# ChanghyeonKim93/nonlinear_optimizer_for_slam

Measured on AMD Instinct MI355X. Metric: ndt6_gauss_newton_residual_blocks_per_sec, higher is better.
Workload: dtype f64

## Files before the change

### nonlinear_optimizer_for_slam_amd/csrc/assemble_indexed.hpp

```cpp
#pragma once

#include "assemble_one_launch.hpp"

namespace nos {

struct IndexedLayout {
  const void* points;
  const int32_t* index;
  const void* table;
  uint64_t n_padded;
};

template <typename T>
__device__ __forceinline__ void load_voxel_record(const T* table, int32_t v, T (&rec)[12]) {
  const T* p = table + size_t(16) * size_t(v);
  if constexpr (sizeof(T) == 8) {
    using V2 = double __attribute__((ext_vector_type(2)));
    const V2* q = reinterpret_cast<const V2*>(p);
#pragma unroll
    for (int k = 0; k < 4; ++k) {
      const V2 t = q[k];
      rec[2 * k] = t[0];
      rec[2 * k + 1] = t[1];
    }
// ... 44 lines not shown
  T pt[kPointRing][3];
  int32_t id[kPointRing][K];
  T rc[kRecordRing][K][12];
  auto evaluate = [&](bool live, const T (&p)[3], const int32_t (&vid)[K], const T (&rec)[K][12]) {
#pragma unroll
    for (int k = 0; k < K; ++k) {
      if (live && vid[k] >= 0) {
        const T mu[3] = {rec[k][0], rec[k][1], rec[k][2]};
        const T U[6] = {rec[k][3], rec[k][4], rec[k][5], rec[k][6], rec[k][7], rec[k][8]};
        Problem::item_U(p, mu, U, P, acc);
      }
    }
  };
  uint32_t c = blockIdx.x;
  const uint32_t g = gridDim.x;
#pragma unroll
  for (int s = 0; s < kPointAhead; ++s) load_point(c + uint32_t(s) * g, pt[s], id[s]);
  load_records(id[0], rc[0]);
  for (; c < n_chunks; c += uint32_t(kUnroll) * g) {
#pragma unroll
    for (int u = 0; u < kUnroll; ++u) {
      load_point(c + uint32_t(u + kPointAhead) * g, pt[(u + kPointAhead) % kPointRing], id[(u + kPointAhead) % kPointRing]);
      load_records(id[(u + 1) % kPointRing], rc[(u + 1) % kRecordRing]);
      __builtin_amdgcn_sched_barrier(0);
      evaluate(c + uint32_t(u) * g < n_chunks, pt[u % kPointRing], id[u % kPointRing], rc[u % kRecordRing]);
      __builtin_amdgcn_sched_barrier(0);
    }
  }
  double dacc[kOut];
#pragma unroll
  for (int k = 0; k < kOut; ++k) dacc[k] = double(acc[k]);
  block_reduce_store<kOut, BLOCK>(dacc, partials + size_t(blockIdx.x) * kOut, fin.write_through != 0);
  if (fin.counter != nullptr) finish_in_last_block<kOut, BLOCK>(partials, fin);
}

template <typename SRC, typename DST>
__global__ __launch_bounds__(256) void gather_plane_kernel(const SRC* __restrict__ src, const uint32_t* __restrict__ perm,
                                                           uint64_t n, uint64_t n_padded, DST pad_value,
                                                           DST* __restrict__ dst) {
  const uint64_t j = uint64_t(blockIdx.x) * 256 + threadIdx.x;
  if (j >= n_padded) return;
  dst[j] = j < n ? DST(src[perm ? perm[j] : j]) : pad_value;
}

template <typename T>
__global__ __launch_bounds__(256) void build_voxel_table_kernel(const double* __restrict__ means,
                                                                const double* __restrict__ sqrt_infos,
                                                                const uint32_t* __restrict__ rows, uint64_t n_voxels,
                                                                T* __restrict__ table) {
  const uint64_t t = uint64_t(blockIdx.x) * 256 + threadIdx.x;
  const uint64_t r = t >> 4;
  const int k = int(t & 15);
  if (r >= n_voxels) return;
  const uint64_t v = rows ? rows[r] : r;
  T val = T(0);
  if (k < 3) {
    val = T(means[3 * v + k]);
  } else if (k < 9) {
    double S[9], U[6];
#pragma unroll
    for (int q = 0; q < 9; ++q) S[q] = sqrt_infos[9 * v + q];
    sqrt_info_to_U<double>(S, U);
    const int q = k - 3;
    val = T(q == 0 ? U[0] : q == 1 ? U[1] : q == 2 ? U[2] : q == 3 ? U[3] : q == 4 ? U[4] : U[5]);
  }
  table[t] = val;
// ... 19 lines not shown
```

### nonlinear_optimizer_for_slam_amd/csrc/nos_core.hip

```cpp
#include "nos_internal.hpp"

namespace nosd {


thread_local const void* t_last_kernel = nullptr;

template <typename Problem, typename T, int ITEMS, int BLOCK, int MINW, int PREFETCH = 0>
int launch_variant(const nos::TiledLayout& L, const typename Problem::Params& P, int grid_cap, int num_cus_hint,
                   bool nt, double* partials, const nos::FusedFinal& fin_in, hipStream_t stream, int* rows_out) {
  constexpr uint32_t kChunk = BLOCK * ITEMS;
  if (L.n_padded % kChunk != 0) return fail(NOS_ERR_INVALID_ARGUMENT, "n_padded %% chunk != 0");
  if (L.tile_stride != 0 && ((size_t(L.tile_mask) + 1) % kChunk) != 0)
    return fail(NOS_ERR_INVALID_ARGUMENT, "tile not a multiple of the kernel chunk");
  const uint64_t n_chunks64 = L.n_padded / kChunk;
  if (n_chunks64 > 0xFFFFFFFFull) return fail(NOS_ERR_UNSUPPORTED, "dataset too large for one shard");
  const uint32_t n_chunks = uint32_t(n_chunks64);
  int grid = int(std::min<uint64_t>(n_chunks, uint64_t(grid_cap)));
  if (grid < 1) grid = 1;
  if (grid > kMaxPartialRows) grid = kMaxPartialRows;
  nos::FusedFinal fin = fin_in;
  fin.write_through = (fin.counter != nullptr && grid <= num_cus_hint && fin_in.write_through != 0) ? 1 : 0;
  const auto kernel = nt ? nos::assemble_kernel<Problem, T, ITEMS, BLOCK, MINW, true, PREFETCH>
                         : nos::assemble_kernel<Problem, T, ITEMS, BLOCK, MINW, false, PREFETCH>;
  t_last_kernel = reinterpret_cast<const void*>(kernel);
// ... 38 lines not shown
  } else {
    if (variant == 0) variant = kReproj ? 11 : 1;
    switch (variant) {
      NOS_CASE(1, 2, 512, 2, 1)
      NOS_CASE_PP(11, 2, 512, 2, 1)
#ifdef NOS_ALL_VARIANTS
      NOS_CASE(2, 1, 256, 4, 2)
      NOS_CASE(3, 2, 256, 5, 2)
      NOS_CASE(4, 2, 256, 4, 2)
      NOS_CASE(5, 1, 1024, 4, 1)
      NOS_CASE(6, 2, 1024, 4, 1)
      NOS_CASE(9, 2, 256, 3, 3)
      NOS_CASE_PP(12, 4, 512, 2, 1)
      NOS_CASE(13, 4, 256, 2, 1)
#endif
    }
  }
#undef NOS_CASE
#undef NOS_CASE_PP
  return fail(NOS_ERR_UNSUPPORTED, "launch geometry %d is not compiled into this build for this element type "
              "(default build: fp64 0, 1, 3, 7; fp32 1, 11; `make ALL_VARIANTS=1` builds the rest)", variant);
}

size_t resident_items_per_lane(int n_fields, int dtype) {
  if (n_fields == 15)
    return dtype == NOS_F64 ? size_t(nos::ResidentShape<15, 8>::RI + nos::ResidentShape<15, 8>::LI)
                            : size_t(nos::ResidentShape<15, 4>::RI + nos::ResidentShape<15, 4>::LI);
  if (n_fields == 5)
    return dtype == NOS_F64 ? size_t(nos::ResidentShape<5, 8>::RI + nos::ResidentShape<5, 8>::LI)
                            : size_t(nos::ResidentShape<5, 4>::RI + nos::ResidentShape<5, 4>::LI);
  return 1;
}

struct SingleBlockArgs {
  int cluster_blocks = 0;
  int items_per_lane = 1;
  int stream_chunks = 0;
  bool nt = false;
  int stream_lds_chunks = 0;
  int stream_reg_rounds = 0;
  bool stage1_sc1 = false;
  const nos::Mailbox* mail = nullptr;
  double* partials = nullptr;
  nos::ClusterCtl* ctl = nullptr;
  nos::LmDevice* lm;
  double* history;
  int history_capacity;
  double* entry;
  unsigned long long* seq_host;
  unsigned long long seq;
};

template <typename Problem, typename T>
int launch_single(const nos::TiledLayout& L, const typename Problem::Params& P, const SingleBlockArgs& a, hipStream_t stream) {
  constexpr int kBlock = 512;
  if (L.n_padded % kBlock != 0) return fail(NOS_ERR_INVALID_ARGUMENT, "n_padded %% 512 != 0");
  if (a.cluster_blocks > 0 && a.stream_chunks > 0) {
    constexpr int kSI = sizeof(T) == 8 ? 1 : 2;
    constexpr bool kSPF = false;
    constexpr size_t kChunk = size_t(kBlock) * kSI;
    if (L.n_padded % kChunk != 0 || (L.tile_stride != 0 && ((size_t(L.tile_mask) + 1) % kChunk) != 0))
      return fail(NOS_ERR_INVALID_ARGUMENT, "streaming solve: layout not a multiple of the %zu-item chunk", kChunk);
    if (size_t(a.stream_chunks) * kChunk != L.n_padded) return fail(NOS_ERR_INVALID_ARGUMENT, "streaming solve: chunk count does not match the layout");
    const auto kernel = a.nt ? nos::solve_cluster_kernel<Problem, T, kBlock, 0, 0, kSI, kSPF, true>
                             : nos::solve_cluster_kernel<Problem, T, kBlock, 0, 0, kSI, kSPF, false>;
    uint32_t lds = uint32_t(std::min(std::max(a.stream_lds_chunks, 0), 3));
    size_t dyn_bytes = lds * size_t(Problem::kFields) * kChunk * sizeof(T);
    if (dyn_bytes > size_t(48) * 1024 &&
        hipFuncSetAttribute(reinterpret_cast<const void*>(kernel), hipFuncAttributeMaxDynamicSharedMemorySize,
                            int(dyn_bytes)) != hipSuccess) {
      (void)hipGetLastError();
      lds = 0;
      dyn_bytes = 0;
    }
    const uint32_t reg = uint32_t(std::min(std::max(a.stream_reg_rounds, 0), nos::kStreamRegRoundsMax));
    t_last_kernel = reinterpret_cast<const void*>(kernel);
    hipLaunchKernelGGL(kernel, dim3(a.cluster_blocks), dim3(kBlock), dyn_bytes, stream, L, P, a.partials, a.lm, a.ctl, a.history,
                       a.history_capacity, a.entry, a.seq_host, a.seq, uint32_t(a.stream_chunks) | (a.stage1_sc1 ? 0x80000000u : 0u),
                       a.mail, lds, reg);
    hipError_t e = hipGetLastError();
    if (e != hipSuccess) return fail(NOS_ERR_HIP, "streaming solve launch failed: %s", hipGetErrorString(e));
    return NOS_OK;
  }
  if (a.cluster_blocks > 0) {
    using Shape = nos::ResidentShape<Problem::kPlanes, int(sizeof(T))>;
// ... 36 lines not shown
  });
}

int check_loss(const nos_loss* loss, int* kind_out) {
  int kind = loss ? loss->kind : NOS_LOSS_NONE;
  if (kind < NOS_LOSS_NONE || kind > NOS_LOSS_HUBER) return fail(NOS_ERR_INVALID_ARGUMENT, "unknown loss kind %d", kind);
  if (kind == NOS_LOSS_EXPONENTIAL && (loss->a < 0.0 || loss->b < 0.0))
    return fail(NOS_ERR_INVALID_ARGUMENT, "exponential loss needs c1 >= 0 and c2 >= 0");
  if (kind == NOS_LOSS_HUBER && !(loss->a > 0.0)) return fail(NOS_ERR_INVALID_ARGUMENT, "huber loss needs threshold > 0");
  *kind_out = kind;
  return NOS_OK;
}

bool use_nontemporal(const nos_dataset* ds, const Shard& sh) {
  const int force = ds->ctx->settings.nt;
  if (force >= 0) return force != 0;
  return sh.bytes > (size_t(192) << 20);
}

template <template <typename, int> class ProblemT, typename T>
int launch_flat(const nos_dataset* ds, const Shard& sh, const Request& rq, double* partials, const nos::FusedFinal& fin,
                hipStream_t stream, int* rows_out, const SingleBlockArgs* single) {
  const nos_ctx* ctx = ds->ctx;
  typename ProblemT<T, nos::kLossNone>::Params P{};
  fill_params(P, rq, ds);
  return launch_by_loss<ProblemT, T>(rq.loss_kind, ctx->variant, ctx->blocks_per_cu, ctx->slots[sh.slot].num_cus, sh.layout, P,
                                     use_nontemporal(ds, sh), partials, fin, stream, rows_out, single);
}

int launch_assemble_inner(const nos_dataset* ds, const Shard& sh, const Request& rq, double* partials,
                          const nos::FusedFinal& fin_in, hipStream_t stream, int* rows_out, const SingleBlockArgs* single) {
  nos::FusedFinal fin = fin_in;
  fin.write_through = ds->ctx->settings.sc1;
  if (ds->kind == kKindNdtIndexed) return launch_indexed(ds, sh, rq, partials, fin, stream, rows_out);
  const bool f64 = ds->dtype == NOS_F64;
  if (rq.problem == 6)
    return f64 ? launch_flat<nos::Ndt6Problem, double>(ds, sh, rq, partials, fin, stream, rows_out, single)
               : launch_flat<nos::Ndt6Problem, float>(ds, sh, rq, partials, fin, stream, rows_out, single);
  if (rq.problem == 3)
    return f64 ? launch_flat<nos::Ndt3Problem, double>(ds, sh, rq, partials, fin, stream, rows_out, single)
               : launch_flat<nos::Ndt3Problem, float>(ds, sh, rq, partials, fin, stream, rows_out, single);
  return f64 ? launch_flat<nos::ReprojProblem, double>(ds, sh, rq, partials, fin, stream, rows_out, single)
             : launch_flat<nos::ReprojProblem, float>(ds, sh, rq, partials, fin, stream, rows_out, single);
}

int launch_assemble_raw(const nos_dataset* ds, const Shard& sh, const Request& rq, double* partials,
                        const nos::FusedFinal& fin_in, hipStream_t stream, int* rows_out,
                        const SingleBlockArgs* single = nullptr) {
  t_last_kernel = nullptr;
  const int rc = launch_assemble_inner(ds, sh, rq, partials, fin_in, stream, rows_out, single);
  if (rc == NOS_OK && t_last_kernel != nullptr) ds->ctx->slots[sh.slot].last_kernel = t_last_kernel;
  return rc;
}

int launch_assemble(const nos_dataset* ds, const Shard& sh, const Request& rq, double* partials,
                    const nos::FusedFinal& fin, hipStream_t stream, int* rows_out) {
  DeviceSlot& slot = ds->ctx->slots[sh.slot];
  if (slot.prof_on && slot.prof_every == 0) ++slot.prof_launches;
  const bool prof = slot.prof_on && slot.prof_every > 0 && (slot.prof_launches++ % slot.prof_every) == 0 &&
                    slot.prof_used + 2 <= slot.prof_events.size();
  if (prof) NOS_HIP_CHECK(hipEventRecord(slot.prof_events[slot.prof_used], stream));
  const int rc = launch_assemble_raw(ds, sh, rq, partials, fin, stream, rows_out);
  if (rc != NOS_OK) return rc;
  if (prof) {
    NOS_HIP_CHECK(hipEventRecord(slot.prof_events[slot.prof_used + 1], stream));
    slot.prof_used += 2;
  }
// ... 258 lines not shown
  const bool with_comm = ctx->comm != nullptr;
  return ds->kind != kKindNdtIndexed && !with_comm && ctx->shm_dev == nullptr && opt->max_iterations > 0 &&
         sh.layout.n * size_t(ds->n_fields) <= nos::kSingleBlockMaxElements && ctx->settings.lm_single != 0 &&
         (opt->cost_history == nullptr || opt->max_iterations <= kHistCapacity);
}

int solve_single_block(nos_dataset* ds, const Request& rq, const nos_lm_options* opt, nos_host::LmState* st) {
  const Shard& sh = ds->shards[0];
  DeviceSlot& slot = ds->ctx->slots[sh.slot];
  SingleBlockArgs single{};
  single.lm = slot.d_lm;
  single.history = opt->cost_history ? slot.h_hist_dev : nullptr;
  single.history_capacity = kHistCapacity;
  single.entry = slot.h_log_dev;
  single.seq_host = reinterpret_cast<unsigned long long*>(slot.h_out_dev + kSeqSlot);
  single.seq = ++slot.seq;
  int rows = 0;
  int rc = launch_assemble_raw(ds, sh, rq, slot.partials, nos::FusedFinal{}, slot.stream, &rows, &single);
  if (rc != NOS_OK) return rc;
  rc = wait_for_sequence(slot, single.seq);
  if (rc != NOS_OK) return rc;
  const double* e = slot.h_log;
  read_log_entry(e, st);
  const int executed = int(e[nos::kLogExecuted]);
  if (slot.prof_on && slot.prof_every == 0) slot.prof_launches += executed;
  copy_history(opt, slot, executed);
  return NOS_OK;
}

bool cluster_eligible(const nos_dataset* ds, const nos_lm_options* opt, bool mailbox_in_launch, size_t cluster_blocks,
                      bool resident_fits, bool stream_form, bool paused) {
  const nos_ctx* ctx = ds->ctx;
  const bool with_comm = ctx->comm != nullptr;
  return ds->kind != kKindNdtIndexed && !with_comm && (ctx->shm_dev == nullptr || mailbox_in_launch) && opt->max_iterations > 0 &&
         cluster_blocks >= 1 && (resident_fits || stream_form) && !paused &&
         ctx->settings.lm_cluster != 0 && (opt->cost_history == nullptr || opt->max_iterations <= kHistCapacity);
}

int solve_cluster(nos_dataset* ds, const Request& rq, const nos_lm_options* opt, const nos::LmInitArgs& init,
                  nos_host::LmState* st, bool* finished, int* fell_back) {
  nos_ctx* ctx = ds->ctx;
  const Shard& sh = ds->shards[0];
  DeviceSlot& slot = ctx->slots[sh.slot];
  *finished = false;
  const size_t max_blocks = std::min<size_t>(std::min<size_t>(nos::kClusterMaxBlocks, size_t(slot.num_cus)),
                                             size_t(std::max(1, ctx->settings.lm_cluster_max_blocks)));
  const bool mailbox_in_launch = ctx->shm_dev != nullptr && ctx->d_peers != nullptr && ctx->d_mail != nullptr &&
                                 ds->kind != kKindNdtIndexed;
  const size_t cluster_blocks = std::min<size_t>(max_blocks, (sh.layout.n + 511) / 512);
  const size_t items_per_lane = cluster_blocks > 0 ? (sh.layout.n + cluster_blocks * 512 - 1) / (cluster_blocks * 512) : 0;
  const size_t resident_capacity = ctx->settings.lm_cluster == 2 ? 1 : resident_items_per_lane(ds->n_fields, ds->dtype);
  const size_t stream_chunk = size_t(512) * (ds->dtype == NOS_F64 ? 1 : 2);
  const bool resident_fits = items_per_lane >= 1 && items_per_lane <= resident_capacity;
  const bool stream_form = !resident_fits && (ctx->settings.lm_cluster == 1 || ctx->settings.lm_cluster == 5) && items_per_lane >= 1 &&
                           sh.layout.n_padded % stream_chunk == 0 && sh.layout.n_padded / stream_chunk < (size_t(1) << 31) &&
                           (sh.layout.tile_stride == 0 || (size_t(sh.layout.tile_mask) + 1) % stream_chunk == 0);
  bool paused = false;
  if (mailbox_in_launch) {
    paused = slot.cluster_paused_solves > 0;
    if (paused) --slot.cluster_paused_solves;
  } else {
    if (slot.cluster_gave_up &&
        std::chrono::steady_clock::now() - slot.cluster_gave_up_at > std::chrono::milliseconds(ctx->settings.lm_cluster_retry_ms))
      slot.cluster_gave_up = false;
    paused = slot.cluster_gave_up;
  }
  if (!cluster_eligible(ds, opt, mailbox_in_launch, cluster_blocks, resident_fits, stream_form, paused)) return NOS_OK;
  SingleBlockArgs cl{};
  cl.cluster_blocks = int(cluster_blocks);
  cl.items_per_lane = int(items_per_lane);
  if (stream_form) {
    cl.items_per_lane = 0;
    cl.stream_chunks = int(sh.layout.n_padded / stream_chunk);
    cl.nt = use_nontemporal(ds, sh);
    cl.stream_lds_chunks = ctx->settings.stream_lds_chunks;
    cl.stream_reg_rounds = ctx->settings.stream_reg_rounds;
  }
  cl.stage1_sc1 = ctx->settings.lm_cluster == 5;
  cl.mail = mailbox_in_launch ? ctx->d_mail : nullptr;
  cl.partials = slot.partials;
  cl.ctl = slot.d_cluster;
  cl.lm = slot.d_lm;
  cl.history = opt->cost_history ? slot.h_hist_dev : nullptr;
  cl.history_capacity = kHistCapacity;
  cl.entry = slot.h_log_dev;
  cl.seq_host = reinterpret_cast<unsigned long long*>(slot.h_out_dev + kSeqSlot);
  cl.seq = ++slot.seq;
  NOS_HIP_CHECK(hipMemsetAsync(slot.d_cluster, 0, sizeof(nos::ClusterCtl), slot.stream));
  if (ctx->settings.debug_cluster_abort != 0) {
    const unsigned int raised = 1u;
    NOS_HIP_CHECK(hipMemcpyAsync(&slot.d_cluster->abort, &raised, sizeof raised, hipMemcpyHostToDevice, slot.stream));
    NOS_HIP_CHECK(hipStreamSynchronize(slot.stream));
  }
  int rows = 0;
  const int rc_launch = launch_assemble_raw(ds, sh, rq, slot.partials, nos::FusedFinal{}, slot.stream, &rows, &cl);
  if (rc_launch != NOS_OK && rc_launch != NOS_ERR_UNSUPPORTED) return rc_launch;
  const bool launched_ok = rc_launch == NOS_OK;
  *finished = launched_ok && spin_for_sequence(slot, cl.seq, 4000000);
  if (!*finished) {
    NOS_HIP_CHECK(hipStreamSynchronize(slot.stream));
    *finished = spin_for_sequence(slot, cl.seq, 1);
  }
  if (*finished) {
    slot.cluster_next_pause = 64;
    const double* e = slot.h_log;
    read_log_entry(e, st);
    const int executed = int(e[nos::kLogExecuted]);
#ifdef NOS_LM_TIMING
    fprintf(stderr, "[resident-timing] %d blocks x %d items/lane (0 = streamed), %d iterations; workgroup 0, us per iteration: item math %.2f, "
            "block reduce %.2f, drain+arrive+wait %.2f, rows->sums %.2f, LM step+barrier %.2f\n", cl.cluster_blocks,
// ... 262 lines not shown
```

### nonlinear_optimizer_for_slam_amd/csrc/nos_ctx.hip

```cpp
#include "nos_internal.hpp"

#include <cxxabi.h>

namespace nosd {

namespace {
thread_local std::string g_last_error;
}

int fail(int status, const char* fmt, ...) {
  char buf[512];
  va_list ap;
  va_start(ap, fmt);
  vsnprintf(buf, sizeof buf, fmt, ap);
  va_end(ap);
  g_last_error = buf;
  return status;
}

const char* last_error_text() { return g_last_error.c_str(); }
void clear_last_error() { g_last_error.clear(); }

std::string dir_of_symbol(const void* symbol, std::string* file_out) {
  Dl_info info{};
// ... 70 lines not shown
struct OptionEntry {
  const char* key;
  int nosd::Settings::*field;
  int lo, hi;
};
const OptionEntry kOptions[] = {
    {"plane_skew", &nosd::Settings::plane_skew, 0, 1 << 20},
    {"sc1", &nosd::Settings::sc1, 0, 1},
    {"nt", &nosd::Settings::nt, -1, 1},
    {"fused", &nosd::Settings::fused, 0, 1},
    {"lm_fused", &nosd::Settings::lm_fused, 0, 1},
    {"lm_window", &nosd::Settings::lm_window, 1, nosd::kLogSlots - 2},
    {"lm_single", &nosd::Settings::lm_single, 0, 1},
    {"lm_cluster", &nosd::Settings::lm_cluster, 0, 5},
    {"lm_cluster_retry_ms", &nosd::Settings::lm_cluster_retry_ms, 0, 3600000},
    {"pool", &nosd::Settings::pool, 0, 1},
    {"tile_log2", &nosd::Settings::tile_log2, -1, 24},
    {"ingest", &nosd::Settings::ingest, 0, 2},
    {"ingest_threads", &nosd::Settings::ingest_threads, 0, 1024},
    {"indexed_bpc", &nosd::Settings::indexed_bpc, 1, 16},
    {"match_dense", &nosd::Settings::match_dense, 0, 1},
    {"map_compact_keys", &nosd::Settings::map_compact_keys, 0, 1},
    {"pgo_host_scalars", &nosd::Settings::pgo_host_scalars, 0, 1},
    {"pgo_precond", &nosd::Settings::pgo_precond, 0, 1},
    {"pgo_agg", &nosd::Settings::pgo_agg, 2, 1 << 20},
    {"pgo_block", &nosd::Settings::pgo_block, 0, 1},
    {"pgo_coarse_probe", &nosd::Settings::pgo_coarse_probe, 0, 1},
    {"map_fma_mask", &nosd::Settings::map_fma_mask, 0, (1 << 26) - 1},
    {"map_eigen_version", &nosd::Settings::map_eigen_version, 33, 34},
    {"debug_cluster_abort", &nosd::Settings::debug_cluster_abort, 0, 2},
    {"lm_cluster_max_blocks", &nosd::Settings::lm_cluster_max_blocks, 1, 256},
    {"stream_lds_chunks", &nosd::Settings::stream_lds_chunks, 0, 3},
    {"stream_reg_rounds", &nosd::Settings::stream_reg_rounds, 0, nos::kStreamRegRoundsMax},
    {"batch_max_elements", &nosd::Settings::batch_max_elements, 0, 1 << 30},
};
bool option_in_range(const OptionEntry& o, int value) {
  if (value < o.lo || value > o.hi) return false;
  if (!strcmp(o.key, "tile_log2")) return value <= 0 || value >= 10;
  return true;
}
void drop_out_of_range_settings(nosd::Settings& st) {
  const nosd::Settings defaults;
  for (const OptionEntry& o : kOptions)
    if (!option_in_range(o, st.*(o.field))) {
      fprintf(stderr, "[nos-hip] NOS_%s = %d is outside [%d, %d]: ignored\n", o.key, st.*(o.field), o.lo, o.hi);
      st.*(o.field) = defaults.*(o.field);
    }
}
}


extern "C" {

int nos_ctx_create(const int* device_ids, int n_devices, nos_ctx** out_ctx) {
  if (!out_ctx) return fail(NOS_ERR_INVALID_ARGUMENT, "out_ctx is NULL");
  *out_ctx = nullptr;
  if (n_devices < 1 || n_devices > 64 || !device_ids) return fail(NOS_ERR_INVALID_ARGUMENT, "bad device list");
  int count = 0;
  hipError_t e = hipGetDeviceCount(&count);
  if (e != hipSuccess || count < 1)
    return fail(NOS_ERR_NO_DEVICE, "no usable HIP device (%s); this library has no CPU fallback",
                e != hipSuccess ? hipGetErrorString(e) : "device count is 0");
  for (int i = 0; i < n_devices; ++i)
    if (device_ids[i] < 0 || device_ids[i] >= count)
      return fail(NOS_ERR_INVALID_ARGUMENT, "device id %d out of range [0,%d)", device_ids[i], count);
  nos_ctx* ctx = new (std::nothrow) nos_ctx();
  if (!ctx) return fail(NOS_ERR_OUT_OF_MEMORY, "host allocation failed");
  ctx->slots.resize(n_devices);
  ctx->blocks_per_cu = env_int("NOS_BLOCKS_PER_CU", 0);
  ctx->variant = env_int("NOS_VARIANT", 0);
  {
    Settings& st = ctx->settings;
    st.plane_skew = env_int("NOS_PLANE_SKEW", st.plane_skew);
    st.sc1 = env_int("NOS_SC1", st.sc1);
    st.nt = env_int("NOS_NT", st.nt);
    st.fused = env_int("NOS_FUSED", st.fused);
    st.lm_fused = env_int("NOS_LM_FUSED", st.lm_fused);
    st.lm_window = env_int("NOS_LM_WINDOW", st.lm_window);
    st.lm_single = env_int("NOS_LM_SINGLE", st.lm_single);
    st.lm_cluster = env_int("NOS_LM_CLUSTER", st.lm_cluster);
    st.lm_cluster_max_blocks = env_int("NOS_LM_CLUSTER_MAX_BLOCKS", st.lm_cluster_max_blocks);
    st.stream_lds_chunks = env_int("NOS_STREAM_LDS_CHUNKS", st.stream_lds_chunks);
    st.stream_reg_rounds = env_int("NOS_STREAM_REG_ROUNDS", st.stream_reg_rounds);
    st.batch_max_elements = env_int("NOS_BATCH_MAX_ELEMENTS", st.batch_max_elements);
    st.pool = env_int("NOS_POOL", st.pool);
    st.tile_log2 = env_int("NOS_TILE_LOG2", st.tile_log2);
    const char* ingest = getenv("NOS_INGEST");
    st.ingest = (ingest && !strcmp(ingest, "pack")) ? 1 : ((ingest && !strcmp(ingest, "unpack")) ? 2 : 0);
    st.ingest_threads = env_int("NOS_INGEST_THREADS", 0);
    st.indexed_bpc = env_int("NOS_INDEXED_BPC", st.indexed_bpc);
    st.match_dense = env_int("NOS_MATCH_DENSE", st.match_dense);
    st.map_compact_keys = env_int("NOS_MAP_COMPACT_KEYS", st.map_compact_keys);
    st.pgo_host_scalars = env_int("NOS_PGO_HOST_SCALARS", st.pgo_host_scalars);
    st.pgo_precond = env_int("NOS_PGO_PRECOND", st.pgo_precond);
    st.pgo_agg = env_int("NOS_PGO_AGG", st.pgo_agg);
    st.pgo_block = env_int("NOS_PGO_BLOCK", st.pgo_block);
    st.pgo_coarse_probe = env_int("NOS_PGO_COARSE_PROBE", st.pgo_coarse_probe);
    drop_out_of_range_settings(st);
  }
  for (int i = 0; i < n_devices; ++i) {
    DeviceSlot& s = ctx->slots[i];
    s.device = device_ids[i];
    s.pool_enabled = ctx->settings.pool != 0;
    hipDeviceProp_t prop;
    e = hipSetDevice(s.device);
    if (e == hipSuccess) e = hipGetDeviceProperties(&prop, s.device);
    if (e == hipSuccess) {
      s.num_cus = prop.multiProcessorCount > 0 ? prop.multiProcessorCount : 256;
      e = hipStreamCreateWithFlags(&s.own_stream, hipStreamNonBlocking);
    }
    if (e == hipSuccess) e = hipMalloc(&s.partials, sizeof(double) * kMaxPartialRows * kMaxOut);
    if (e == hipSuccess) e = hipMalloc(&s.d_out, sizeof(double) * kMaxOut);
    if (e == hipSuccess) e = hipHostMalloc(&s.h_out, sizeof(double) * 64, hipHostMallocMapped);
    if (e == hipSuccess) memset(s.h_out, 0, sizeof(double) * 64);
    if (e == hipSuccess) e = hipHostGetDevicePointer(reinterpret_cast<void**>(&s.h_out_dev), s.h_out, 0);
    if (e == hipSuccess) e = hipMalloc(&s.d_lm, sizeof(nos::LmDevice));
// ... 252 lines not shown
```

### nonlinear_optimizer_for_slam_amd/csrc/nos_indexed.hip

```cpp
#define NOS_WITH_MATCH_INDEX_KERNEL
#include "group_host.hpp"
#include "match_host.hpp"

using namespace nosd;

namespace {

template <typename Problem, typename T, int K>
int launch_indexed_kernel(const nos::IndexedLayout& L, const typename Problem::Params& P, int grid_cap, int num_cus,
                          double* partials, const nos::FusedFinal& fin_in, hipStream_t stream, int* rows_out) {
  constexpr int kBlock = sizeof(T) == 8 ? 512 : 768;
  constexpr int kMinWaves = sizeof(T) == 8 ? 2 : 3;
  const uint64_t n_chunks64 = L.n_padded / kBlock;
  if (n_chunks64 > 0xFFFFFFFFull) return fail(NOS_ERR_UNSUPPORTED, "dataset too large for one shard");
  int grid = int(std::min<uint64_t>(std::max<uint64_t>(n_chunks64, 1), uint64_t(grid_cap)));
  if (grid > kMaxPartialRows) grid = kMaxPartialRows;
  nos::FusedFinal fin = fin_in;
  fin.write_through = (fin.counter != nullptr && grid <= num_cus && fin_in.write_through != 0) ? 1 : 0;
  hipLaunchKernelGGL((nos::assemble_indexed_kernel<Problem, T, K, kBlock, kMinWaves>), dim3(grid), dim3(kBlock), 0, stream, L,
                     P, uint32_t(n_chunks64), partials, fin);
  hipError_t e = hipGetLastError();
  if (e != hipSuccess) return fail(NOS_ERR_HIP, "indexed assemble launch failed: %s", hipGetErrorString(e));
  *rows_out = grid;
  return NOS_OK;
}

template <template <typename, int> class ProblemT, typename T, typename ParamsT>
int launch_indexed_by_loss(int loss_kind, int n_slots, const nos::IndexedLayout& L, const ParamsT& P, int grid_cap,
                           int num_cus, double* partials, const nos::FusedFinal& fin, hipStream_t stream, int* rows_out) {
  return with_loss(loss_kind, [&](auto loss) {
    using Problem = ProblemT<T, decltype(loss)::value>;
    return n_slots == 1 ? launch_indexed_kernel<Problem, T, 1>(L, P, grid_cap, num_cus, partials, fin, stream, rows_out)
                        : launch_indexed_kernel<Problem, T, 2>(L, P, grid_cap, num_cus, partials, fin, stream, rows_out);
  });
}

template <template <typename, int> class ProblemT, typename T>
int launch_indexed_problem(const nos_dataset* ds, const Shard& sh, const Request& rq, double* partials,
                           const nos::FusedFinal& fin, hipStream_t stream, int* rows_out) {
  const nos_ctx* ctx = ds->ctx;
  const DeviceSlot& slot = ctx->slots[sh.slot];
  nos::IndexedLayout L{};
  L.points = sh.data;
  L.index = sh.index;
  L.table = sh.table;
  L.n_padded = sh.layout.n_padded;
  typename ProblemT<T, nos::kLossNone>::Params P{};
  fill_params(P, rq, ds);
  return launch_indexed_by_loss<ProblemT, T>(rq.loss_kind, sh.n_slots, L, P, ctx->settings.indexed_bpc * slot.num_cus,
                                             slot.num_cus, partials, fin, stream, rows_out);
}

}

int nosd::launch_indexed(const nos_dataset* ds, const Shard& sh, const Request& rq, double* partials,
                         const nos::FusedFinal& fin, hipStream_t stream, int* rows_out) {
  const bool f64 = ds->dtype == NOS_F64;
  if (rq.problem == 6)
    return f64 ? launch_indexed_problem<nos::Ndt6Problem, double>(ds, sh, rq, partials, fin, stream, rows_out)
               : launch_indexed_problem<nos::Ndt6Problem, float>(ds, sh, rq, partials, fin, stream, rows_out);
  if (rq.problem == 3)
    return f64 ? launch_indexed_problem<nos::Ndt3Problem, double>(ds, sh, rq, partials, fin, stream, rows_out)
               : launch_indexed_problem<nos::Ndt3Problem, float>(ds, sh, rq, partials, fin, stream, rows_out);
  return fail(NOS_ERR_WRONG_KIND, "voxel-indexed datasets serve the NDT entry points only");
}

int nosd::indexed_from_device(nos_ctx* ctx, size_t n, const double* d_points, int n_slots, const int32_t* d_index,
                              size_t n_voxels, const double* d_means, const double* d_sqrt_infos, const uint32_t* d_rows,
                              int dtype, int sort_by_voxel, nos_dataset** out_ds) {
  if (dtype != NOS_F64 && dtype != NOS_F32) return fail(NOS_ERR_INVALID_ARGUMENT, "unknown dtype %d", dtype);
  if (n >= 0xFFFFFFFFull) return fail(NOS_ERR_UNSUPPORTED, "too many points for one indexed dataset");
  nos_dataset* ds = new (std::nothrow) nos_dataset();
  if (!ds) return fail(NOS_ERR_OUT_OF_MEMORY, "host allocation failed");
  ds->ctx = ctx;
  ds->kind = kKindNdtIndexed;
  ds->dtype = dtype;
  ds->n_fields = 3;
  ds->n = n;
  ds->shards.resize(1);
  Shard& sh = ds->shards[0];
  sh.slot = 0;
  sh.n_slots = n_slots;
  sh.n_voxels = n_voxels;
  const size_t pad = 3072;
  const size_t n_padded = std::max<size_t>(((n + pad - 1) / pad) * pad, pad);
  sh.layout.n = n;
  sh.layout.n_padded = n_padded;
  sh.layout.tile_stride = 0;
  sh.layout.field_stride = n_padded;
  sh.layout.tile_shift = 40;
  sh.layout.tile_mask = 0xFFFFFFFFu;
  const size_t es = elem_size(dtype);
  sh.bytes = n_padded * (3 * es + sizeof(int32_t) * size_t(n_slots));
  DeviceSlot& slot = ctx->slots[0];
  hipStream_t st = slot.stream;
  DeviceBuffers tmp(&slot);
// ... 165 lines not shown
```

### nonlinear_optimizer_for_slam_amd/csrc/nos_internal.hpp

```cpp
#pragma once

#include <hip/hip_runtime.h>
#include <dlfcn.h>
#include <fcntl.h>
#include <sys/mman.h>
#include <sys/stat.h>
#include <unistd.h>
#include <rccl/rccl.h>

#include <algorithm>
#include <atomic>
#include <chrono>
#include <random>
#include <climits>
#include <cmath>
#include <cstdarg>
#include <cstdio>
#include <cstdlib>
#include <cstring>
#include <map>
#include <memory>
#include <new>
#include <string>
#include <thread>
// ... 106 lines not shown
  int prof_every = 1;
  long prof_launches = 0;
};

constexpr int kMapReferenceFmaMask = (4 | 8 | 16 | 32) | ((1 | 4 | 8 | 32 | 256) << 8) | (0x1ff << 17);
struct Settings {
  int plane_skew = 1088;
  int sc1 = 1;
  int nt = -1;
  int fused = 1;
  int lm_fused = 1;
  int lm_window = 3;
  int lm_single = 1;
  int lm_cluster_retry_ms = 5000;
  int lm_cluster = 1;
  int pool = 1;
  int tile_log2 = -1;
  int ingest = 0;
  int ingest_threads = 0;
  int indexed_bpc = 1;
  int match_dense = 1;
  int map_compact_keys = 1;
  int pgo_host_scalars = 0;
  int pgo_precond = 1;
  int pgo_agg = 48;
  int pgo_coarse_probe = 0;
  int pgo_block = 1;
  int map_fma_mask = kMapReferenceFmaMask;
  int map_eigen_version = 34;
  int debug_cluster_abort = 0;
  int lm_cluster_max_blocks = 256;
  int stream_lds_chunks = 3;
  int stream_reg_rounds = 3;
  int batch_max_elements = int(nos::kSingleBlockMaxElements);
};
}

struct nos_ctx {
  std::recursive_mutex mu;
  nosd::Settings settings;
  std::vector<nosd::DeviceSlot> slots;
  int blocks_per_cu = 0;
  int variant = 0;
  int tile_log2 = -1;
  ncclComm_t comm = nullptr;
  int comm_ranks = 1;
  int comm_rank = 0;
  void* shm_host = nullptr;
  size_t shm_bytes = 0;
  double* shm_dev = nullptr;
  unsigned long long* d_round = nullptr;
  nos::Mailbox* d_mail = nullptr;
  double* ipc_own = nullptr;
  std::vector<double*> ipc_peers;
  double** d_peers = nullptr;
};

namespace nosd {

struct CtxGuard {
  std::unique_lock<std::recursive_mutex> lock;
  explicit CtxGuard(const nos_ctx* ctx) {
    if (ctx != nullptr) lock = std::unique_lock<std::recursive_mutex>(const_cast<nos_ctx*>(ctx)->mu);
  }
};

// ... 231 lines not shown
                             const uint32_t* seg_count, uint32_t n_voxels, double inv_res, double res, double* acc_out,
                             hipStream_t stream);
struct LiveStore {
  nos_ctx* ctx;
  nos::VoxelMatchView view;
  unsigned long long* d_count;
  unsigned int* d_error;
  double span;
  bool broken;
};
inline int check_live_store(const LiveStore& s) {
  if (s.span > double(nos::kVoxelMatchMaxSpan))
    return fail(NOS_ERR_UNSUPPORTED,
                "the search ball spans more than %d voxel cells per axis (2 r / resolution + 2 = %g): match against a snapshot",
                nos::kVoxelMatchMaxSpan, s.span);
  if (s.broken) return fail(NOS_ERR_HIP, "the voxel store was left undefined by an earlier failure");
  return NOS_OK;
}
inline int check_scans(const nos_ctx* ctx, nos_scan* const* scans, int n) {
  for (int i = 0; i < n; ++i) {
    if (scans[i] == nullptr) return fail(NOS_ERR_INVALID_ARGUMENT, "scan %d is NULL", i);
    if (scans[i]->ctx != ctx) return fail(NOS_ERR_INVALID_ARGUMENT, "scan %d belongs to another context than the map", i);
  }
  return NOS_OK;
}
int register_live(int dof, const LiveStore* store, nos_scan* const* scans, int32_t n_problems, double* R, double* t,
                  const nos_loss* loss, const nos_register_options* ropt, const nos_lm_options* options,
                  nos_register_report* reports);
int score_live(const LiveStore* store, nos_scan* const* scans, int32_t n_problems, const double* R, const double* t,
               const nos_loss* loss, int max_neighbors, nos_pose_score* scores);
int indexed_from_device(nos_ctx* ctx, size_t n, const double* d_points, int n_slots, const int32_t* d_index, size_t n_voxels,
                        const double* d_means, const double* d_sqrt_infos, const uint32_t* d_rows, int dtype,
                        int sort_by_voxel, nos_dataset** out_ds);
int launch_indexed(const nos_dataset* ds, const Shard& sh, const Request& rq, double* partials,
                   const nos::FusedFinal& fin, hipStream_t stream, int* rows_out);

}
```

Before: 76.99 billion.

## Run indexed NDT Gauss-Newton solve as one persistent cluster kernel with LDS-resident points

Adds a persistent cluster kernel for voxel-indexed NDT datasets. It runs every LM iteration inside one launch, using a tagged two-stage cross-block all-reduce and an on-device LM step, so the per-iteration kernel launches and host round trips go away. On the first iteration it also caches as many point coordinates and voxel indices in LDS as fit, so later iterations read them from LDS instead of global memory. The cost is a grid limited to co-resident blocks, spin-wait synchronisation with a timeout and abort path, and large dynamic LDS use that may reduce occupancy.

Measured after the change: 76.86 billion. Within noise of the previous version (-0.2%).

```diff
diff --git a/nonlinear_optimizer_for_slam_amd/csrc/assemble_indexed.hpp b/nonlinear_optimizer_for_slam_amd/csrc/assemble_indexed.hpp
--- a/nonlinear_optimizer_for_slam_amd/csrc/assemble_indexed.hpp
+++ b/nonlinear_optimizer_for_slam_amd/csrc/assemble_indexed.hpp
@@ -100,6 +100,282 @@
   for (int k = 0; k < kOut; ++k) dacc[k] = double(acc[k]);
   block_reduce_store<kOut, BLOCK>(dacc, partials + size_t(blockIdx.x) * kOut, fin.write_through != 0);
   if (fin.counter != nullptr) finish_in_last_block<kOut, BLOCK>(partials, fin);
+}
+
+template <typename T, int K, int BLOCK>
+constexpr size_t indexed_round_bytes() {
+  return size_t(BLOCK) * (3 * sizeof(T) + K * sizeof(int32_t));
+}
+
+template <typename Problem, typename T, int K, int BLOCK>
+__global__ __launch_bounds__(BLOCK) void solve_indexed_cluster_kernel(IndexedLayout L, typename Problem::Params P,
+                                                                     uint32_t n_chunks, uint32_t lds_rounds,
+                                                                     uint32_t stage1_sc1, double* __restrict__ partials,
+                                                                     LmDevice* lm, ClusterCtl* ctl,
+                                                                     double* __restrict__ cost_history, int history_capacity,
+                                                                     double* entry_host, unsigned long long* seq_host,
+                                                                     unsigned long long seq) {
+  constexpr int kOut = Problem::kOut;
+  constexpr int kCols = 32;
+  constexpr int kSlices = BLOCK / kCols;
+  static_assert(kSlices >= 8, "stage 2 of the all-reduce reads eight group rows at once");
+  const T* __restrict__ pts = static_cast<const T*>(L.points);
+  const T* __restrict__ table = static_cast<const T*>(L.table);
+  extern __shared__ __align__(16) unsigned char indexed_resident_raw[];
+  __shared__ int s_flag;
+  __shared__ int s_fast;
+  __shared__ double red[kSlices][kCols];
+  __shared__ double s_tot[kLmTotDoubles(kOut)];
+  __shared__ double s_lmd_raw[(sizeof(LmDevice) + 7) / 8];
+  LmDevice& s_lmd = *reinterpret_cast<LmDevice*>(s_lmd_raw);
+  nos_host::LmState& s_state = s_lmd.st;
+
+  const uint32_t g = gridDim.x;
+  const uint32_t my_rounds = blockIdx.x < n_chunks ? (n_chunks - blockIdx.x + g - 1u) / g : 0u;
+  const uint32_t res_k = min(lds_rounds, my_rounds);
+  auto lds_plane = [&](uint32_t r, int f) -> T* {
+    return reinterpret_cast<T*>(indexed_resident_raw + size_t(r) * indexed_round_bytes<T, K, BLOCK>()) + size_t(f) * BLOCK + threadIdx.x;
+  };
+  auto lds_ids = [&](uint32_t r, int k) -> int32_t* {
+    return reinterpret_cast<int32_t*>(indexed_resident_raw + size_t(r) * indexed_round_bytes<T, K, BLOCK>() +
+                                      size_t(3) * BLOCK * sizeof(T)) + size_t(k) * BLOCK + threadIdx.x;
+  };
+
+  const uint32_t last_chunk = n_chunks - 1u;
+  auto load_point = [&](uint32_t c, T (&p)[3], int32_t (&vid)[K]) {
+    const uint64_t i = uint64_t(c < n_chunks ? c : last_chunk) * BLOCK + threadIdx.x;
+    p[0] = __builtin_nontemporal_load(pts + i);
+    p[1] = __builtin_nontemporal_load(pts + L.n_padded + i);
+    p[2] = __builtin_nontemporal_load(pts + 2 * L.n_padded + i);
+#pragma unroll
+    for (int k = 0; k < K; ++k) vid[k] = __builtin_nontemporal_load(L.index + uint64_t(k) * L.n_padded + i);
+  };
+  auto load_records = [&](const int32_t (&vid)[K], T (&rec)[K][12]) {
+#pragma unroll
+    for (int k = 0; k < K; ++k) load_voxel_record<T>(table, vid[k] < 0 ? 0 : vid[k], rec[k]);
+  };
+  constexpr int kPointAhead = sizeof(T) == 8 ? 4 : 3, kPointRing = kPointAhead + 1, kRecordRing = 2,
+                kUnroll = (kPointRing % kRecordRing == 0) ? kPointRing : kPointRing * kRecordRing;
+  T pt[kPointRing][3];
+  int32_t id[kPointRing][K];
+  T rc[kRecordRing][K][12];
+  T acc[kOut];
+  auto evaluate = [&](bool live, const T (&p)[3], const int32_t (&vid)[K], const T (&rec)[K][12]) {
+#pragma unroll
+    for (int k = 0; k < K; ++k) {
+      if (live && vid[k] >= 0) {
+        const T mu[3] = {rec[k][0], rec[k][1], rec[k][2]};
+        const T U[6] = {rec[k][3], rec[k][4], rec[k][5], rec[k][6], rec[k][7], rec[k][8]};
+        Problem::item_U(p, mu, U, P, acc);
+      }
+    }
+  };
+  auto evaluate_lds = [&](uint32_t r, const int32_t (&vid)[K], const T (&rec)[K][12]) {
+    const T p[3] = {*lds_plane(r, 0), *lds_plane(r, 1), *lds_plane(r, 2)};
+    evaluate(true, p, vid, rec);
+  };
+
+#pragma unroll
+  for (int s = 0; s < kPointAhead; ++s) load_point(blockIdx.x + uint32_t(s) * g, pt[s], id[s]);
+  if (threadIdx.x == 0) {
+    s_lmd.settings = lm->settings;
+    s_state = lm->st;
+    s_flag = s_state.done != 0 ? 1 : 0;
+    s_fast = 0;
+    if (__hip_atomic_load(&ctl->abort, __ATOMIC_RELAXED, __HIP_MEMORY_SCOPE_AGENT) != 0u) s_flag = 2;
+  }
+  __syncthreads();
+  const unsigned int n_groups = g < 8u ? g : 8u;
+  const bool allow_fast = stage1_sc1 == 0u;
+  constexpr int kXccCol = 28;
+  const unsigned int my_xcc = xcc_id();
+  unsigned int it = 0;
+  int executed = 0;
+  while (s_flag == 0) {
+    set_pose(P, &s_lmd);
+#pragma unroll
+    for (int k = 0; k < kOut; ++k) acc[k] = T(0);
+    const bool fill = it == 0u;
+    const uint32_t first = fill ? 0u : res_k;
+    if (first == 0u) {
+      load_records(id[0], rc[0]);
+    } else {
+      int32_t la[K], lb[K];
+#pragma unroll
+      for (int k = 0; k < K; ++k) la[k] = *lds_ids(0u, k);
+      load_records(la, rc[0]);
+      for (uint32_t r = 0;; r += 2u) {
+        const bool more_a = r + 1u < first;
+#pragma unroll
+        for (int k = 0; k < K; ++k) {
+          const int32_t v = *lds_ids(more_a ? r + 1u : r, k);
+          lb[k] = more_a ? v : id[0][k];
+        }
+        load_records(lb, rc[1]);
+        __builtin_amdgcn_sched_barrier(0);
+        evaluate_lds(r, la, rc[0]);
+        __builtin_amdgcn_sched_barrier(0);
+        if (!more_a) {
+#pragma unroll
+          for (int k = 0; k < K; ++k)
+#pragma unroll
+            for (int m = 0; m < 9; ++m) rc[0][k][m] = rc[1][k][m];
+          break;
+        }
+        const bool more_b = r + 2u < first;
+#pragma unroll
+        for (int k = 0; k < K; ++k) {
+          const int32_t v = *lds_ids(more_b ? r + 2u : r, k);
+          la[k] = more_b ? v : id[0][k];
+        }
+        load_records(la, rc[0]);
+        __builtin_amdgcn_sched_barrier(0);
+        evaluate_lds(r + 1u, lb, rc[1]);
+        __builtin_amdgcn_sched_barrier(0);
+        if (!more_b) break;
+      }
+    }
+    for (uint32_t c = blockIdx.x + first * g, round = first; c < n_chunks; c += uint32_t(kUnroll) * g, round += uint32_t(kUnroll)) {
+#pragma unroll
+      for (int u = 0; u < kUnroll; ++u) {
+        load_point(c + uint32_t(u + kPointAhead) * g, pt[(u + kPointAhead) % kPointRing], id[(u + kPointAhead) % kPointRing]);
+        load_records(id[(u + 1) % kPointRing], rc[(u + 1) % kRecordRing]);
+        __builtin_amdgcn_sched_barrier(0);
+        if (fill && round + uint32_t(u) < res_k) {
+#pragma unroll
+          for (int f = 0; f < 3; ++f) *lds_plane(round + uint32_t(u), f) = pt[u % kPointRing][f];
+#pragma unroll
+          for (int k = 0; k < K; ++k) *lds_ids(round + uint32_t(u), k) = id[u % kPointRing][k];
+        }
+        evaluate(c + uint32_t(u) * g < n_chunks, pt[u % kPointRing], id[u % kPointRing], rc[u % kRecordRing]);
+        __builtin_amdgcn_sched_barrier(0);
+      }
+    }
+    if (res_k < my_rounds) {
+      uint32_t next_first = res_k;
+      asm volatile("" : "+s"(next_first));
+#pragma unroll
+      for (int s = 0; s < kPointAhead; ++s) load_point(blockIdx.x + (next_first + uint32_t(s)) * g, pt[s], id[s]);
+    }
+    double dacc[kOut];
+#pragma unroll
+    for (int k = 0; k < kOut; ++k) dacc[k] = double(acc[k]);
+    {
+      double* rows = partials;
+      asm volatile("" : "+s"(rows));
+      TaggedUnit* const block_units = reinterpret_cast<TaggedUnit*>(rows);
+      TaggedUnit* const group_units = block_units + size_t(kClusterMaxBlocks) * 32;
+      const unsigned long long tag = (seq << 24) | ((unsigned long long)it + 1ull);
+      const double mine = block_reduce_value<kOut, BLOCK>(dacc);
+      const bool probe = it == 0u && allow_fast;
+      if (threadIdx.x < kOut) {
+        if (s_fast != 0)
+          tagged_store_plain(block_units + size_t(blockIdx.x) * 32 + threadIdx.x, mine, tag);
+        else
+          tagged_store(block_units + size_t(blockIdx.x) * 32 + threadIdx.x, mine, tag);
+      } else if (probe && threadIdx.x == kXccCol) {
+        tagged_store(block_units + size_t(blockIdx.x) * 32 + kXccCol, double(my_xcc), tag);
+      }
+      const unsigned long long deadline = wall_clock64() + kClusterTimeoutTicks;
+      auto await = [&](const TaggedUnit* u, double* value) -> bool {
+        unsigned int polls = 0;
+        for (;;) {
+          const TaggedUnit got = tagged_load(u);
+          if (got.seq == tag) {
+            *value = got.value;
+            return true;
+          }
+          if ((++polls & 63u) == 0u &&
+              (__hip_atomic_load(&ctl->abort, __ATOMIC_RELAXED, __HIP_MEMORY_SCOPE_AGENT) != 0u || wall_clock64() > deadline)) {
+            __hip_atomic_store(&ctl->abort, 1u, __ATOMIC_RELAXED, __HIP_MEMORY_SCOPE_AGENT);
+            s_flag = 2;
+            return false;
+          }
+        }
+      };
+      const int col = threadIdx.x % kCols;
+      const int slice = threadIdx.x / kCols;
+      if (blockIdx.x < n_groups) {
+        const unsigned int g_size = (g - blockIdx.x + 7u) >> 3;
+        double gsum = 0.0;
+        for (unsigned int m0 = 0; m0 < g_size; m0 += kSlices) {
+          const unsigned int m = m0 + slice;
+          double v = 0.0;
+          if (m < g_size && (col < kOut || (probe && col == kXccCol))) {
+            (void)await(block_units + size_t(blockIdx.x + 8u * m) * 32 + col, &v);
+            if (col == kXccCol) v = v == double(my_xcc) ? 0.0 : 1.0;
+          }
+          red[slice][col] = v;
+          __syncthreads();
+          if (threadIdx.x < kOut || (probe && threadIdx.x == kXccCol)) {
+#pragma unroll
+            for (int sl = 0; sl < kSlices; ++sl) gsum += red[sl][threadIdx.x];
+          }
+          __syncthreads();
+        }
+        if ((threadIdx.x < kOut || (probe && threadIdx.x == kXccCol)) && s_flag != 2)
+          tagged_store(group_units + (size_t(it & 1u) * 8 + blockIdx.x) * 32 + threadIdx.x, gsum, tag);
+      }
+      {
+        double v = 0.0;
+        if (slice < int(n_groups) && (col < kOut || (probe && col == kXccCol)) && s_flag != 2)
+          (void)await(group_units + (size_t(it & 1u) * 8 + slice) * 32 + col, &v);
+        if (slice < 8) red[slice][col] = v;
+      }
+      __syncthreads();
+      if (s_flag == 2) break;
+      if (threadIdx.x < kOut) {
+        double tot = 0.0;
+        for (unsigned int gr = 0; gr < n_groups; ++gr) tot += red[gr][threadIdx.x];
+        s_tot[threadIdx.x] = tot;
+      } else if (probe && threadIdx.x == kXccCol) {
+        double strangers = 0.0;
+        for (unsigned int gr = 0; gr < n_groups; ++gr) strangers += red[gr][kXccCol];
+        s_fast = strangers == 0.0 ? 1 : 0;
+      }
+      __syncthreads();
+    }
+    if (threadIdx.x == 0) {
+      if (blockIdx.x == 0 && cost_history != nullptr && executed < history_capacity)
+        __hip_atomic_store(cost_history + executed, s_tot[kOut - 1], __ATOMIC_RELAXED, __HIP_MEMORY_SCOPE_SYSTEM);
+      lm_step_lane<kOut>(lds_ptr(s_tot), lds_ptr(&s_lmd));
+      s_flag = s_state.done != 0 ? 1 : 0;
+    }
+    ++executed;
+    ++it;
+    __syncthreads();
+  }
+  if (s_flag == 1 && blockIdx.x == 0) {
+    if (threadIdx.x < kOut && entry_host != nullptr && executed > 0)
+      __hip_atomic_store(entry_host + kLogOut + threadIdx.x, s_tot[threadIdx.x], __ATOMIC_RELAXED, __HIP_MEMORY_SCOPE_SYSTEM);
+    if (threadIdx.x == 0) {
+      const nos_host::LmState st = s_state;
+      lm->st = st;
+      if (entry_host != nullptr) {
+#pragma unroll
+        for (int k = 0; k < 9; ++k)
+          __hip_atomic_store(entry_host + kLogR + k, st.R[k], __ATOMIC_RELAXED, __HIP_MEMORY_SCOPE_SYSTEM);
+#pragma unroll
+        for (int k = 0; k < 3; ++k)
+          __hip_atomic_store(entry_host + kLogT + k, st.t[k], __ATOMIC_RELAXED, __HIP_MEMORY_SCOPE_SYSTEM);
+        __hip_atomic_store(entry_host + kLogLambda, st.lambda, __ATOMIC_RELAXED, __HIP_MEMORY_SCOPE_SYSTEM);
+        __hip_atomic_store(entry_host + kLogPrevCost, st.previous_cost, __ATOMIC_RELAXED, __HIP_MEMORY_SCOPE_SYSTEM);
+        __hip_atomic_store(entry_host + kLogCost, st.cost, __ATOMIC_RELAXED, __HIP_MEMORY_SCOPE_SYSTEM);
+        __hip_atomic_store(entry_host + kLogIteration, double(st.iteration), __ATOMIC_RELAXED, __HIP_MEMORY_SCOPE_SYSTEM);
+        __hip_atomic_store(entry_host + kLogDone, double(st.done), __ATOMIC_RELAXED, __HIP_MEMORY_SCOPE_SYSTEM);
+        __hip_atomic_store(entry_host + kLogOk, double(st.ok), __ATOMIC_RELAXED, __HIP_MEMORY_SCOPE_SYSTEM);
+        __hip_atomic_store(entry_host + kLogExecuted, double(executed), __ATOMIC_RELAXED, __HIP_MEMORY_SCOPE_SYSTEM);
+      }
+    }
+    if (threadIdx.x < kWave) {
+      asm volatile("s_waitcnt vmcnt(0)" ::: "memory");
+      if (threadIdx.x == 0 && seq_host != nullptr) {
+        __builtin_amdgcn_fence(__ATOMIC_RELEASE, "");
+        asm volatile("s_waitcnt vmcnt(0)" ::: "memory");
+        __hip_atomic_store(seq_host, seq, __ATOMIC_RELAXED, __HIP_MEMORY_SCOPE_SYSTEM);
+      }
+    }
+  }
 }
 
 template <typename SRC, typename DST>
diff --git a/nonlinear_optimizer_for_slam_amd/csrc/nos_core.hip b/nonlinear_optimizer_for_slam_amd/csrc/nos_core.hip
--- a/nonlinear_optimizer_for_slam_amd/csrc/nos_core.hip
+++ b/nonlinear_optimizer_for_slam_amd/csrc/nos_core.hip
@@ -94,25 +94,6 @@
   return 1;
 }
 
-struct SingleBlockArgs {
-  int cluster_blocks = 0;
-  int items_per_lane = 1;
-  int stream_chunks = 0;
-  bool nt = false;
-  int stream_lds_chunks = 0;
-  int stream_reg_rounds = 0;
-  bool stage1_sc1 = false;
-  const nos::Mailbox* mail = nullptr;
-  double* partials = nullptr;
-  nos::ClusterCtl* ctl = nullptr;
-  nos::LmDevice* lm;
-  double* history;
-  int history_capacity;
-  double* entry;
-  unsigned long long* seq_host;
-  unsigned long long seq;
-};
-
 template <typename Problem, typename T>
 int launch_single(const nos::TiledLayout& L, const typename Problem::Params& P, const SingleBlockArgs& a, hipStream_t stream) {
   constexpr int kBlock = 512;
@@ -215,7 +196,7 @@
                           const nos::FusedFinal& fin_in, hipStream_t stream, int* rows_out, const SingleBlockArgs* single) {
   nos::FusedFinal fin = fin_in;
   fin.write_through = ds->ctx->settings.sc1;
-  if (ds->kind == kKindNdtIndexed) return launch_indexed(ds, sh, rq, partials, fin, stream, rows_out);
+  if (ds->kind == kKindNdtIndexed) return launch_indexed(ds, sh, rq, partials, fin, stream, rows_out, single);
   const bool f64 = ds->dtype == NOS_F64;
   if (rq.problem == 6)
     return f64 ? launch_flat<nos::Ndt6Problem, double>(ds, sh, rq, partials, fin, stream, rows_out, single)
@@ -540,7 +521,7 @@
                       bool resident_fits, bool stream_form, bool paused) {
   const nos_ctx* ctx = ds->ctx;
   const bool with_comm = ctx->comm != nullptr;
-  return ds->kind != kKindNdtIndexed && !with_comm && (ctx->shm_dev == nullptr || mailbox_in_launch) && opt->max_iterations > 0 &&
+  return !with_comm && (ctx->shm_dev == nullptr || mailbox_in_launch) && opt->max_iterations > 0 &&
          cluster_blocks >= 1 && (resident_fits || stream_form) && !paused &&
          ctx->settings.lm_cluster != 0 && (opt->cost_history == nullptr || opt->max_iterations <= kHistCapacity);
 }
@@ -555,11 +536,12 @@
                                              size_t(std::max(1, ctx->settings.lm_cluster_max_blocks)));
   const bool mailbox_in_launch = ctx->shm_dev != nullptr && ctx->d_peers != nullptr && ctx->d_mail != nullptr &&
                                  ds->kind != kKindNdtIndexed;
-  const size_t cluster_blocks = std::min<size_t>(max_blocks, (sh.layout.n + 511) / 512);
+  const bool indexed = ds->kind == kKindNdtIndexed;
+  const size_t cluster_blocks = indexed ? (sh.layout.n > 0 ? max_blocks : 0) : std::min<size_t>(max_blocks, (sh.layout.n + 511) / 512);
   const size_t items_per_lane = cluster_blocks > 0 ? (sh.layout.n + cluster_blocks * 512 - 1) / (cluster_blocks * 512) : 0;
   const size_t resident_capacity = ctx->settings.lm_cluster == 2 ? 1 : resident_items_per_lane(ds->n_fields, ds->dtype);
   const size_t stream_chunk = size_t(512) * (ds->dtype == NOS_F64 ? 1 : 2);
-  const bool resident_fits = items_per_lane >= 1 && items_per_lane <= resident_capacity;
+  const bool resident_fits = !indexed && items_per_lane >= 1 && items_per_lane <= resident_capacity;
   const bool stream_form = !resident_fits && (ctx->settings.lm_cluster == 1 || ctx->settings.lm_cluster == 5) && items_per_lane >= 1 &&
                            sh.layout.n_padded % stream_chunk == 0 && sh.layout.n_padded / stream_chunk < (size_t(1) << 31) &&
                            (sh.layout.tile_stride == 0 || (size_t(sh.layout.tile_mask) + 1) % stream_chunk == 0);
@@ -584,6 +566,7 @@
     cl.stream_lds_chunks = ctx->settings.stream_lds_chunks;
     cl.stream_reg_rounds = ctx->settings.stream_reg_rounds;
   }
+  cl.indexed_lds_rounds = ctx->settings.indexed_lds_rounds;
   cl.stage1_sc1 = ctx->settings.lm_cluster == 5;
   cl.mail = mailbox_in_launch ? ctx->d_mail : nullptr;
   cl.partials = slot.partials;
diff --git a/nonlinear_optimizer_for_slam_amd/csrc/nos_ctx.hip b/nonlinear_optimizer_for_slam_amd/csrc/nos_ctx.hip
--- a/nonlinear_optimizer_for_slam_amd/csrc/nos_ctx.hip
+++ b/nonlinear_optimizer_for_slam_amd/csrc/nos_ctx.hip
@@ -126,6 +126,7 @@
     {"lm_cluster_max_blocks", &nosd::Settings::lm_cluster_max_blocks, 1, 256},
     {"stream_lds_chunks", &nosd::Settings::stream_lds_chunks, 0, 3},
     {"stream_reg_rounds", &nosd::Settings::stream_reg_rounds, 0, nos::kStreamRegRoundsMax},
+    {"indexed_lds_rounds", &nosd::Settings::indexed_lds_rounds, -1, 1024},
     {"batch_max_elements", &nosd::Settings::batch_max_elements, 0, 1 << 30},
 };
 bool option_in_range(const OptionEntry& o, int value) {
@@ -176,6 +177,7 @@
     st.lm_cluster_max_blocks = env_int("NOS_LM_CLUSTER_MAX_BLOCKS", st.lm_cluster_max_blocks);
     st.stream_lds_chunks = env_int("NOS_STREAM_LDS_CHUNKS", st.stream_lds_chunks);
     st.stream_reg_rounds = env_int("NOS_STREAM_REG_ROUNDS", st.stream_reg_rounds);
+    st.indexed_lds_rounds = env_int("NOS_INDEXED_LDS_ROUNDS", st.indexed_lds_rounds);
     st.batch_max_elements = env_int("NOS_BATCH_MAX_ELEMENTS", st.batch_max_elements);
     st.pool = env_int("NOS_POOL", st.pool);
     st.tile_log2 = env_int("NOS_TILE_LOG2", st.tile_log2);
diff --git a/nonlinear_optimizer_for_slam_amd/csrc/nos_indexed.hip b/nonlinear_optimizer_for_slam_amd/csrc/nos_indexed.hip
--- a/nonlinear_optimizer_for_slam_amd/csrc/nos_indexed.hip
+++ b/nonlinear_optimizer_for_slam_amd/csrc/nos_indexed.hip
@@ -25,11 +25,53 @@
   return NOS_OK;
 }
 
+template <typename Problem, typename T, int K>
+int launch_indexed_cluster(const nos::IndexedLayout& L, const typename Problem::Params& P, int device, const SingleBlockArgs& a,
+                           hipStream_t stream) {
+  constexpr int kBlock = 512;
+  const auto kernel = nos::solve_indexed_cluster_kernel<Problem, T, K, kBlock>;
+  const uint64_t n_chunks64 = L.n_padded / kBlock;
+  if (L.n_padded % kBlock != 0 || n_chunks64 < 1) return fail(NOS_ERR_INVALID_ARGUMENT, "indexed solve: n_padded %% 512 != 0");
+  if (n_chunks64 >= (uint64_t(1) << 31)) return fail(NOS_ERR_UNSUPPORTED, "dataset too large for one shard");
+  const int grid = int(std::min<uint64_t>(n_chunks64, uint64_t(std::min(std::max(a.cluster_blocks, 1), int(nos::kClusterMaxBlocks)))));
+  static std::atomic<int> static_lds{-1};
+  int fixed = static_lds.load(std::memory_order_relaxed);
+  if (fixed < 0) {
+    hipFuncAttributes fa{};
+    NOS_HIP_CHECK(hipFuncGetAttributes(&fa, reinterpret_cast<const void*>(kernel)));
+    fixed = int(fa.sharedSizeBytes);
+    static_lds.store(fixed, std::memory_order_relaxed);
+  }
+  int lds_max = 0;
+  NOS_HIP_CHECK(hipDeviceGetAttribute(&lds_max, hipDeviceAttributeMaxSharedMemoryPerBlock, device));
+  constexpr size_t kRound = nos::indexed_round_bytes<T, K, kBlock>();
+  const size_t room = size_t(std::max(lds_max - ((fixed + 15) & ~15), 0));
+  const uint64_t rounds_per_block = (n_chunks64 + uint64_t(grid) - 1) / uint64_t(grid);
+  uint64_t rounds = std::min<uint64_t>(room / kRound, rounds_per_block);
+  if (a.indexed_lds_rounds >= 0) rounds = std::min<uint64_t>(rounds, uint64_t(a.indexed_lds_rounds));
+  const size_t dyn_bytes = size_t(rounds) * kRound;
+  if (dyn_bytes > size_t(48) * 1024) {
+    const hipError_t ea = hipFuncSetAttribute(reinterpret_cast<const void*>(kernel), hipFuncAttributeMaxDynamicSharedMemorySize,
+                                              int(dyn_bytes));
+    if (ea != hipSuccess) return fail(NOS_ERR_UNSUPPORTED, "indexed solve: %zu bytes of LDS refused: %s", dyn_bytes, hipGetErrorString(ea));
+  }
+  t_last_kernel = reinterpret_cast<const void*>(kernel);
+  hipLaunchKernelGGL(kernel, dim3(grid), dim3(kBlock), dyn_bytes, stream, L, P, uint32_t(n_chunks64), uint32_t(rounds),
+                     a.stage1_sc1 ? 1u : 0u, a.partials, a.lm, a.ctl, a.history, a.history_capacity, a.entry, a.seq_host, a.seq);
+  hipError_t e = hipGetLastError();
+  if (e != hipSuccess) return fail(NOS_ERR_HIP, "indexed solve launch failed: %s", hipGetErrorString(e));
+  return NOS_OK;
+}
+
 template <template <typename, int> class ProblemT, typename T, typename ParamsT>
 int launch_indexed_by_loss(int loss_kind, int n_slots, const nos::IndexedLayout& L, const ParamsT& P, int grid_cap,
-                           int num_cus, double* partials, const nos::FusedFinal& fin, hipStream_t stream, int* rows_out) {
+                           int num_cus, int device, double* partials, const nos::FusedFinal& fin, hipStream_t stream,
+                           int* rows_out, const SingleBlockArgs* single) {
   return with_loss(loss_kind, [&](auto loss) {
     using Problem = ProblemT<T, decltype(loss)::value>;
+    if (single != nullptr)
+      return n_slots == 1 ? launch_indexed_cluster<Problem, T, 1>(L, P, device, *single, stream)
+                          : launch_indexed_cluster<Problem, T, 2>(L, P, device, *single, stream);
     return n_slots == 1 ? launch_indexed_kernel<Problem, T, 1>(L, P, grid_cap, num_cus, partials, fin, stream, rows_out)
                         : launch_indexed_kernel<Problem, T, 2>(L, P, grid_cap, num_cus, partials, fin, stream, rows_out);
   });
@@ -37,7 +79,7 @@
 
 template <template <typename, int> class ProblemT, typename T>
 int launch_indexed_problem(const nos_dataset* ds, const Shard& sh, const Request& rq, double* partials,
-                           const nos::FusedFinal& fin, hipStream_t stream, int* rows_out) {
+                           const nos::FusedFinal& fin, hipStream_t stream, int* rows_out, const SingleBlockArgs* single) {
   const nos_ctx* ctx = ds->ctx;
   const DeviceSlot& slot = ctx->slots[sh.slot];
   nos::IndexedLayout L{};
@@ -48,20 +90,20 @@
   typename ProblemT<T, nos::kLossNone>::Params P{};
   fill_params(P, rq, ds);
   return launch_indexed_by_loss<ProblemT, T>(rq.loss_kind, sh.n_slots, L, P, ctx->settings.indexed_bpc * slot.num_cus,
-                                             slot.num_cus, partials, fin, stream, rows_out);
+                                             slot.num_cus, slot.device, partials, fin, stream, rows_out, single);
 }
 
 }
 
 int nosd::launch_indexed(const nos_dataset* ds, const Shard& sh, const Request& rq, double* partials,
-                         const nos::FusedFinal& fin, hipStream_t stream, int* rows_out) {
+                         const nos::FusedFinal& fin, hipStream_t stream, int* rows_out, const SingleBlockArgs* single) {
   const bool f64 = ds->dtype == NOS_F64;
   if (rq.problem == 6)
-    return f64 ? launch_indexed_problem<nos::Ndt6Problem, double>(ds, sh, rq, partials, fin, stream, rows_out)
-               : launch_indexed_problem<nos::Ndt6Problem, float>(ds, sh, rq, partials, fin, stream, rows_out);
+    return f64 ? launch_indexed_problem<nos::Ndt6Problem, double>(ds, sh, rq, partials, fin, stream, rows_out, single)
+               : launch_indexed_problem<nos::Ndt6Problem, float>(ds, sh, rq, partials, fin, stream, rows_out, single);
   if (rq.problem == 3)
-    return f64 ? launch_indexed_problem<nos::Ndt3Problem, double>(ds, sh, rq, partials, fin, stream, rows_out)
-               : launch_indexed_problem<nos::Ndt3Problem, float>(ds, sh, rq, partials, fin, stream, rows_out);
+    return f64 ? launch_indexed_problem<nos::Ndt3Problem, double>(ds, sh, rq, partials, fin, stream, rows_out, single)
+               : launch_indexed_problem<nos::Ndt3Problem, float>(ds, sh, rq, partials, fin, stream, rows_out, single);
   return fail(NOS_ERR_WRONG_KIND, "voxel-indexed datasets serve the NDT entry points only");
 }
 
diff --git a/nonlinear_optimizer_for_slam_amd/csrc/nos_internal.hpp b/nonlinear_optimizer_for_slam_amd/csrc/nos_internal.hpp
--- a/nonlinear_optimizer_for_slam_amd/csrc/nos_internal.hpp
+++ b/nonlinear_optimizer_for_slam_amd/csrc/nos_internal.hpp
@@ -162,6 +162,7 @@
   int lm_cluster_max_blocks = 256;
   int stream_lds_chunks = 3;
   int stream_reg_rounds = 3;
+  int indexed_lds_rounds = -1;
   int batch_max_elements = int(nos::kSingleBlockMaxElements);
 };
 }
@@ -459,7 +460,27 @@
 int indexed_from_device(nos_ctx* ctx, size_t n, const double* d_points, int n_slots, const int32_t* d_index, size_t n_voxels,
                         const double* d_means, const double* d_sqrt_infos, const uint32_t* d_rows, int dtype,
                         int sort_by_voxel, nos_dataset** out_ds);
+struct SingleBlockArgs {
+  int cluster_blocks = 0;
+  int items_per_lane = 1;
+  int stream_chunks = 0;
+  bool nt = false;
+  int stream_lds_chunks = 0;
+  int stream_reg_rounds = 0;
+  int indexed_lds_rounds = -1;
+  bool stage1_sc1 = false;
+  const nos::Mailbox* mail = nullptr;
+  double* partials = nullptr;
+  nos::ClusterCtl* ctl = nullptr;
+  nos::LmDevice* lm;
+  double* history;
+  int history_capacity;
+  double* entry;
+  unsigned long long* seq_host;
+  unsigned long long seq;
+};
+extern thread_local const void* t_last_kernel;
 int launch_indexed(const nos_dataset* ds, const Shard& sh, const Request& rq, double* partials,
-                   const nos::FusedFinal& fin, hipStream_t stream, int* rows_out);
-
-}
+                   const nos::FusedFinal& fin, hipStream_t stream, int* rows_out, const SingleBlockArgs* single = nullptr);
+
+}
```
